# PixelClear/OclPathTracer

Measured on AMD Instinct MI355X. Metric: Msamples/sec (pixels x spp / s), cornellbox.bin 1024x1024, higher is better.
Workload: dtype f32; 1 GPU; BASELINE configs[2]: cornellbox.bin 1024x1024, 256 spp, depth 16, full path; render_lanes=2, checkpointed_launches=True, staging_ring_bytes=402653184, workspace_bytes=510711120

## Files before the change

### include/pt_shim.h

```cpp
#ifndef PT_SHIM_H
#define PT_SHIM_H

#include <stddef.h>
#include <stdint.h>

#ifdef __cplusplus
extern "C" {
#endif

#define PT_SHIM_ABI_VERSION 2

enum pt_status {
    PT_OK = 0,
    PT_ERR_INVALID = 1,
    PT_ERR_NO_DEVICE = 2,
    PT_ERR_OOM = 3,
    PT_ERR_HIP = 4,
    PT_ERR_NOT_FOUND = 5,
    PT_ERR_ARGS = 6,
    PT_ERR_RANGE = 7,
    PT_ERR_TRAVERSAL = 8
};

typedef struct pt_device_s* pt_device_t;
// ... 368 lines not shown
                 const pt_reproject_params* params, const pt_camera* prev_cam, const pt_camera* cur_cam ,
                 pt_event_t ev);

enum { PT_PROF_TRACE = 0, PT_PROF_FOLD = 1, PT_PROF_KINDS = 2 };
int pt_profile_enable(pt_device_t dev, int on);
int pt_profile_query(pt_device_t dev, int kind, double* total_ms, uint64_t* launches);
int pt_profile_query_union(pt_device_t dev, int kind, double* union_ms);
int pt_profile_reset(pt_device_t dev);

#define PT_BVH_SNAPSHOT_BIG_MAX 64
typedef struct pt_bvh_info {
    uint32_t records;
    int32_t num_big;
    int32_t num_triangles;
    float grid_min[3], grid_step[3];
    int32_t reserved[7];
} pt_bvh_info;
int pt_bvh_snapshot(pt_device_t dev, pt_bvh_info* info, void* records, size_t record_capacity, int32_t* big_indices);

int pt_primary_mask_snapshot(pt_device_t dev, uint32_t* num_pixels, void* masks, size_t capacity);

int pt_secondary_mask_snapshot(pt_device_t dev, uint32_t info[4], void* masks, size_t capacity);

int pt_assemble_stripes(pt_device_t dev, pt_buffer_t gathered, pt_buffer_t image, int width,
                        int height, int stripe_rows, int n_ranks, int slab_rows, pt_event_t ev);

int pt_assemble_stripes_on(pt_device_t dev, pt_buffer_t gathered, pt_buffer_t image, int width, int height,
                           int stripe_rows, int n_ranks, int slab_rows, void* hip_stream);

int pt_tonemap_ppm(pt_device_t dev, pt_buffer_t framebuffer, pt_buffer_t rgb_i32, size_t num_pixels,
                   pt_event_t ev);

#ifdef __cplusplus
}
#endif
#endif
```

### oclpathtracer_amd/csrc/pt_kernels.h

```cpp
#pragma once

#include <hip/hip_runtime.h>
#include <stddef.h>
#include <stdint.h>

struct PtRawTriangle { float p1[4], p2[4], p3[4]; int32_t id; char pad[12]; };
struct PtRawMaterial { float albedo[4], emissive[4]; float roughness; int32_t type; char pad[24]; };
static_assert(sizeof(PtRawTriangle) == 64 && sizeof(PtRawMaterial) == 64, "record layout");

struct PtPrepTriangle {
    float p1[3];
    float e1[3];
    float e2[3];
    float pad0[3];
    float n[3];
    int32_t id;
};
static_assert(sizeof(PtPrepTriangle) == 64, "prep layout");

struct PtBvhNode {
    float lmin[3]; uint32_t link_l;
    float lmax[3]; uint32_t link_r;
    float rmin[3]; uint32_t pad0;
    float rmax[3]; uint32_t pad1;
// ... 51 lines not shown
    uint32_t rad1_off;
    int32_t max_bounces, ntri, nmat;
    int32_t stripe_rows, n_ranks, rank;
    uint32_t npix_local;
    uint32_t batches_per_frame, total_batches;
    uint32_t batch;
    float quad_delta1;
    float ray_radius;
    const float* p1tab;
    float p1_lo, p1_hi;
    const PtBvh8Node* bvh;
    int32_t bvh_records;
    PtBvhGrid grid;
    const PtPrepTriangle* bigtab;
    const int32_t* bigidx;
    int32_t nbig;
    const uint2* pmask;
    unsigned int* bvh_flags;
    int32_t bvh_stack_limit;
    uint32_t* carry;
    uint32_t carry_in_waves;
    uint32_t carry_out;
    PtCamera cam;
    const uint2* smask;
};
#define PT_QUEUE_SHARDS 8
#define PT_QUEUE_SHARD_WORDS 1056
#define PT_QUEUE_STOP_WORD (PT_QUEUE_SHARDS * PT_QUEUE_SHARD_WORDS)
#define PT_QUEUE_WORDS ((PT_QUEUE_SHARDS + 1) * PT_QUEUE_SHARD_WORDS)
#define PT_POOL 56
#define PT_CARRY_RECORDS 64
#define PT_CARRY_STRIDE_DW (16 + PT_CARRY_RECORDS * 15)
#define PT_CARRY_HIT_RECORDS PT_POOL
#define PT_CARRY_HIT_STRIDE_DW (16 + PT_CARRY_HIT_RECORDS * 18)
static_assert(PT_CARRY_HIT_STRIDE_DW >= PT_CARRY_STRIDE_DW, "a checkpoint region holds either kernel's records");
static_assert(PT_CARRY_HIT_STRIDE_DW % 4 == 0 && PT_CARRY_STRIDE_DW % 4 == 0, "a region's float4 arrays begin 16 dwords in: every region 16-byte aligned");
#define PT_PACKED_BOUNCE_MAX 256

struct PtFoldParams {
    const float* rad;
    float4* fb;
    uint32_t npix_local;
    int32_t frame_begin, frame_count;
    unsigned int* reset_counter;
    unsigned int* reset_counter2;
};

#define PT_PREP_WORDS 12
__host__ __device__ static inline unsigned ptk_order_key(float f)
{
    unsigned u;
    __builtin_memcpy(&u, &f, sizeof u);
    return (u & 0x80000000u) ? ~u : (u | 0x80000000u);
}
__host__ __device__ static inline float ptk_order_float(unsigned k)
{
    const unsigned u = (k & 0x80000000u) ? (k & 0x7fffffffu) : ~k;
    float f;
    __builtin_memcpy(&f, &u, sizeof f);
    return f;
}
hipError_t ptk_prep_triangles(const PtRawTriangle* raw, PtPrepTriangle* out, int ntri, unsigned int* det_bound_bits,
                              hipStream_t s);
hipError_t ptk_prep_quad_margins(PtPrepTriangle* out, int ntri, float diameter, float delta1, float* p1tab, const float anchor[3], hipStream_t s);
#define PT_P1_STRIDE 24
static inline size_t ptk_p1tab_floats(int ntri) { return (size_t)((ntri / 2 + 1) / 2) * PT_P1_STRIDE; }
hipError_t ptk_primary_masks(const PtTraceParams& p, hipStream_t s);
hipError_t ptk_secondary_masks(const PtPrepTriangle* tris, int ntri, uint2* table, hipStream_t s);
struct PtSearchMode {
    bool bvh;
    bool det_bounded;
    int quads;
};
hipError_t ptk_trace(const PtTraceParams& p, int num_blocks, PtSearchMode m, bool tally, bool wide, hipStream_t s);
#define PT_BVH_NEAR_EYE 4.0f
hipError_t ptk_bvh_big_raw(const PtRawTriangle* raw, const int* bigidx, int nbig, PtRawTriangle* out, hipStream_t s);
static inline size_t ptk_bvh_record_count(int ntri) { return 2 * (size_t)(ntri > 0 ? ntri : 0); }
size_t ptk_bvh_temp_bytes(int ntri);
#define PT_BVH_BIG_MAX 64
#define PT_BVH_RAY_EPS 1.2e-4f
hipError_t ptk_bvh_build(const PtRawTriangle* raw, const PtPrepTriangle* prep, int ntri, PtBvh8Node* recs,
                         PtPrepTriangle* bigtab, int* bigidx, int* nbig_dev, PtBvhGrid* grid_dev, unsigned* used_dev, void* temp, size_t temp_bytes,
                         hipStream_t s);
#define PT_DET_BOUND_MAX 2.0e19f
#define PT_BVH_AUTO_MIN 512
hipError_t ptk_fold(const PtFoldParams& p, hipStream_t s);
hipError_t ptk_assemble_stripes(const float4* gathered, float4* image, int width, int height, int stripe_rows,
                                int n_ranks, int slab_rows, hipStream_t s);
hipError_t ptk_tonemap_ppm(const float4* fb, int32_t* rgb, size_t npix, hipStream_t s);
hipError_t ptk_fill_i32(int32_t* dst, int32_t value, int n, hipStream_t s);
hipError_t ptk_math(const float* in, float* out, int n, hipStream_t s);
// ... 167 lines not shown
```

### oclpathtracer_amd/csrc/pt_kernels.hip

```cpp
#include "pt_kernels.h"

#include "pt_device_math.h"
#include "pt_secmask.h"

#include <type_traits>
#include <utility>

typedef const __attribute__((address_space(4))) float* pt_const_f32p;

PTK_DEV unsigned pt_lane_id() { return __builtin_amdgcn_mbcnt_hi(~0u, __builtin_amdgcn_mbcnt_lo(~0u, 0u)); }
PTK_DEV unsigned pt_mbcnt(unsigned long long m) { return __builtin_amdgcn_mbcnt_hi((unsigned)(m >> 32), __builtin_amdgcn_mbcnt_lo((unsigned)m, 0u)); }

typedef const __attribute__((address_space(4))) PtTraceParams* pt_kargs_p;
PTK_DEV pt_kargs_p pt_kargs()
{
    pt_kargs_p k = (pt_kargs_p)__builtin_amdgcn_kernarg_segment_ptr();
    asm volatile("" : "+s"(k));
    return k;
}
PTK_DEV f3 pt_anchor()
{
    const pt_kargs_p K = pt_kargs();
    return mk3(K->cam.eye[0], K->cam.eye[1], K->cam.eye[2]);
}
// ... 220 lines not shown
    for (int j = 0; j < P.ntri; ++j) {
        const PtPrepTriangle* t = P.tris + j;
        const f3 e1 = mk3(t->e1[0], t->e1[1], t->e1[2]), e2 = mk3(t->e2[0], t->e2[1], t->e2[2]);
        const f3 tv = mk3(o.x - t->p1[0], o.y - t->p1[1], o.z - t->p1[2]);
        const f3 Kd = cross3(e2, e1), Ku = cross3(e2, tv), qv = cross3(tv, e1);
        const float tn = dot3(e2, qv);
        const float detc = dot3(dc, Kd), unc = dot3(dc, Ku), vnc = dot3(dc, qv);
        const float a1 = pt_norm1(e1), a2 = pt_norm1(e2), at = pt_norm1(tv);
        const float rho_d = (eps * pt_norm1(Kd) + uS * (a1 * a2)) * 1.001f + A;
        const float rho_u = (eps * pt_norm1(Ku) + uS * (at * a2)) * 1.001f + A;
        const float rho_v = (eps * pt_norm1(qv) + uS * (at * a1)) * 1.001f + A;
        const bool keep = !(detc + rho_d < 0.999e-8f)
                        & !(unc + rho_u < 0.0f)
                        & !(vnc + rho_v < 0.0f)
                        & !((unc - rho_u) + (vnc - rho_v) > (detc + rho_d) * 1.000002f)
                        & !(tn <= 0.0f);
        const int c = j >> 5;
        const int nc = P.ntri - 32 * c < 32 ? P.ntri - 32 * c : 32;
        m[c] |= (keep ? 1u : 0u) << (nc - 1 - (j & 31));
    }
    P.out[lp] = make_uint2(m[0], m[1]);
}

__global__ __launch_bounds__(256) void pt_secondary_mask_kernel(const PtPrepTriangle* tris, int ntri, uint2* table)
{
    const unsigned i = blockIdx.x * blockDim.x + threadIdx.x;
    if (i < (unsigned)ntri) reinterpret_cast<PtSmTri*>(table)[i] = pt_sm_tri_record(tris[i].p1, tris[i].e1, tris[i].e2);
    if (i >= (unsigned)ntri * PT_SM_TRI_ENTRIES) return;
    const unsigned k = i / PT_SM_TRI_ENTRIES, within = i - k * PT_SM_TRI_ENTRIES;
    const unsigned dir = within / (PT_SM_T * PT_SM_T), tile = within - dir * (PT_SM_T * PT_SM_T);
    const unsigned e = k * PT_SM_TRI_ENTRIES + tile * PT_SM_DIRS + dir;
    const PtSmMask m = pt_sm_entry(reinterpret_cast<const float*>(tris), ntri, e);
    table[PT_SM_HEAD_ENTRIES + e] = make_uint2(m.x, m.y);
}

struct PtTriRec { float p1x, p1y, p1z, e1x, e1y, e1z, e2x, e2y, e2z; };

PTK_DEV PtTriRec pt_load_tri(pt_const_f32p T, int i)
{
    pt_const_f32p t = T + 16 * i;
    PtTriRec r;
    r.p1x = t[0]; r.p1y = t[1]; r.p1z = t[2];
    r.e1x = t[3]; r.e1y = t[4]; r.e1z = t[5];
    r.e2x = t[6]; r.e2y = t[7]; r.e2z = t[8];
    return r;
}

#ifndef PT_VALIDATE_FILTER
#define PT_VALIDATE_FILTER 0
#endif
typedef unsigned long long pt_lanes;
#define PT_LANES(cond) __builtin_amdgcn_ballot_w64(cond)
#define PT_ON(mask) __builtin_amdgcn_inverse_ballot_w64(mask)
PTK_DEV unsigned pt_push_flag(unsigned m, pt_lanes c)
{
    unsigned long long carry_out;
// ... 1068 lines not shown
            if (primary && P.pmask != nullptr) {
                pm = P.pmask[pix0 + lane];
                masked = true;
            } else if (LDS_TABLE == 1 && PT_TRACE_SECONDARY_MASKS && !fresh) {
                const pt_kargs_p KS = pt_kargs();
                const uint2* const sm = KS->smask;
                const int nt = KS->ntri;
                if (sm != nullptr) {
#if PT_STAMPS
                    unsigned long long ta = 0, tb = 0;
                    PT_STAMP(ta);
#endif
                    const PtSmMask ones = pt_sm_all_ones(nt);
                    pm = make_uint2(ones.x, ones.y);
                    if (PT_ON(alive)) {
                        const char* const base = reinterpret_cast<const char*>(sm);
                        const unsigned k = (unsigned)h.hidx < (unsigned)(nt - 1) ? (unsigned)h.hidx : (unsigned)(nt - 1);
                        const float4 ra = *reinterpret_cast<const float4*>(base + (size_t)(k * 48u));
                        const float4 rb = *reinterpret_cast<const float4*>(base + (size_t)(k * 48u + 16u));
                        const float4 rn = *reinterpret_cast<const float4*>(base + (size_t)(k * 48u + 32u));
                        const float A[4] = { ra.x, ra.y, ra.z, ra.w }, B[4] = { rb.x, rb.y, rb.z, rb.w }, N[4] = { rn.x, rn.y, rn.z, rn.w };
                        unsigned entry;
                        const bool covered = pt_sm_classify(A, B, N, s.o.x, s.o.y, s.o.z, s.d.x, s.d.y, s.d.z, k, &entry);
                        const uint2 v = *reinterpret_cast<const uint2*>(base + (size_t)(entry * 8u + (unsigned)(PT_SM_HEAD_ENTRIES * 8)));
                        if (covered) pm = v;
#if PT_VALIDATE_FILTER
                        if (P.stats) {
                            const pt_lanes unc = PT_LANES(!covered);
                            if (lane == (unsigned)__builtin_ctzll(alive)) {
                                atomicAdd(&P.stats[10], (unsigned long long)__popcll(alive));
                                atomicAdd(&P.stats[11], (unsigned long long)__popcll(unc & alive));
                            }
                        }
#endif
                    }
                    masked = true;
#if PT_STAMPS
                    PT_STAMP(tb);
                    c_p1 += tb - ta;
#endif
                }
            }
        }
        if (alive == 0ull) {
        } else if (masked)
            p2steps = pt_intersect_masked<DET_BOUNDED, LDS_TABLE>(T, P.tris, ntri, s.o, s.d, PT_ON(alive), tmax, hu, hv, hidx, pm, tl, lane,
                                                                  PT_VALIDATE_FILTER && P.stats ? P.stats + 2 : nullptr);
// ... 2671 lines not shown
    const int pairs = ntri / 2;
    hipLaunchKernelGGL(pt_prep_quad_margins_kernel, dim3((pairs + 255) / 256), dim3(256), 0, s, out, ntri, diameter, delta1);
    if (p1tab) {
        const int qpairs = (pairs + 1) / 2;
        hipLaunchKernelGGL(pt_prep_p1tab_kernel, dim3((qpairs + 255) / 256), dim3(256), 0, s, out, ntri, diameter, p1tab, anchor[0], anchor[1], anchor[2]);
    }
    return hipGetLastError();
}

hipError_t ptk_primary_masks(const PtTraceParams& p, hipStream_t s)
{
    if (!p.pmask || p.npix_local == 0) return hipSuccess;
    PtMaskParams m;
    m.tris = p.tris;
    m.out = const_cast<uint2*>(p.pmask);
    m.width = p.width; m.height = p.height; m.ntri = p.ntri;
    m.stripe_rows = p.stripe_rows; m.n_ranks = p.n_ranks; m.rank = p.rank;
    m.npix_local = p.npix_local;
    m.cam = p.cam;
    hipLaunchKernelGGL(pt_primary_mask_kernel, dim3((p.npix_local + 255u) / 256u), dim3(256), 0, s, m);
    return hipGetLastError();
}

hipError_t ptk_secondary_masks(const PtPrepTriangle* tris, int ntri, uint2* table, hipStream_t s)
{
    if (!table || ntri <= 0 || ntri > PT_SM_TRI_MAX) return hipErrorInvalidValue;
    const unsigned n = (unsigned)ntri * PT_SM_TRI_ENTRIES;
    hipLaunchKernelGGL(pt_secondary_mask_kernel, dim3((n + 255u) / 256u), dim3(256), 0, s, tris, ntri, table);
    return hipGetLastError();
}

hipError_t ptk_trace(const PtTraceParams& p, int num_blocks, PtSearchMode m, bool tally, bool wide, hipStream_t s)
{
    const bool q3 = m.quads == 3;
    void (*kernel)(const PtTraceParams);
    if (m.bvh && wide)
        kernel = tally ? (m.det_bounded ? (q3 ? pt_trace_bvh_kernel<true, true, 3, true> : pt_trace_bvh_kernel<true, true, 0, true>) : pt_trace_bvh_kernel<false, true, 0, true>)
                       : (m.det_bounded ? (q3 ? pt_trace_bvh_kernel<true, false, 3, true> : pt_trace_bvh_kernel<true, false, 0, true>) : pt_trace_bvh_kernel<false, false, 0, true>);
    else if (m.bvh)
        kernel = tally ? (m.det_bounded ? (q3 ? pt_trace_bvh_kernel<true, true, 3> : pt_trace_bvh_kernel<true, true, 0>) : pt_trace_bvh_kernel<false, true, 0>)
                       : (m.det_bounded ? (q3 ? pt_trace_bvh_kernel<true, false, 3> : pt_trace_bvh_kernel<true, false, 0>) : pt_trace_bvh_kernel<false, false, 0>);
    else if (p.ntri <= PT_LDS_TRI_MAX)
        kernel = m.det_bounded ? (q3 ? pt_trace_kernel<true, 1, 3> : pt_trace_kernel<true, 1, 0>) : pt_trace_kernel<false, 1, 0>;
    else
        kernel = m.det_bounded ? pt_trace_tiled_kernel<true> : pt_trace_tiled_kernel<false>;
    const size_t lds = m.bvh ? ptk_trace_bvh_lds_bytes() : ptk_trace_lds_bytes(p.ntri);
    hipLaunchKernelGGL(kernel, dim3(num_blocks), dim3(PT_TRACE_THREADS), lds, s, p);
    return hipGetLastError();
}

hipError_t ptk_fold(const PtFoldParams& p, hipStream_t s)
// ... 278 lines not shown
```

### oclpathtracer_amd/csrc/pt_secmask.h

```cpp
#pragma once

#include <math.h>
#include <stdint.h>

#if defined(__HIPCC__)
#define PT_SM_HD __host__ __device__ static inline
#else
#define PT_SM_HD static inline
#endif

#ifndef PT_SM_T
#define PT_SM_T 12
#endif
#ifndef PT_SM_C
#define PT_SM_C 11
#endif
#ifndef PT_SM_DEPTH
#define PT_SM_DEPTH 3
#endif
#ifndef PT_SM_BUDGET
#define PT_SM_BUDGET 96
#endif
#ifndef PT_SM_SEP_DET
#define PT_SM_SEP_DET 1e-4
#endif
#define PT_SM_GUARD (1.0 / 64.0)
#define PT_SM_DIRS (6 * PT_SM_C * PT_SM_C)
#define PT_SM_TRI_ENTRIES (PT_SM_T * PT_SM_T * PT_SM_DIRS)
#define PT_SM_TRI_MAX 64
struct PtSmTri { float A[4], B[4], N[4]; };
#define PT_SM_HEAD_ENTRIES (PT_SM_TRI_MAX * sizeof(PtSmTri) / 8)
#define PT_SM_TABLE_BYTES(ntri) ((PT_SM_HEAD_ENTRIES + (size_t)(ntri) * PT_SM_TRI_ENTRIES) * 8)
static_assert(PT_SM_T >= 1 && PT_SM_C >= 1 && PT_SM_C <= 16, "pt_sm_classify's rounding bound is derived for C <= 16");
static_assert(PT_SM_TABLE_BYTES(PT_SM_TRI_MAX) < 0x100000000ull, "an entry's byte offset in the largest table must fit 32 bits");

struct PtSmMask { unsigned x, y; };

PT_SM_HD float pt_sm_form(const float* F, float ox, float oy, float oz)
{
    return __builtin_fmaf(F[2], oz, __builtin_fmaf(F[1], oy, __builtin_fmaf(F[0], ox, F[3])));
}

PT_SM_HD bool pt_sm_classify(const float* A, const float* B, const float* N, float ox, float oy, float oz, float dx, float dy, float dz,
                             unsigned k, unsigned* entry)
{
    const float tu = pt_sm_form(A, ox, oy, oz), tv = pt_sm_form(B, ox, oy, oz), th = pt_sm_form(N, ox, oy, oz);
    const float dd = __builtin_fmaf(dz, dz, __builtin_fmaf(dy, dy, dx * dx));
    const bool covered = (tu >= 0.0f) & (tu < (float)PT_SM_T) & (tv >= 0.0f) & (tv < (float)PT_SM_T) & (__builtin_fabsf(th) <= 1.0f) &
                         (dd >= 0.999f) & (dd <= 1.001f);
    const float ax = __builtin_fabsf(dx), ay = __builtin_fabsf(dy), az = __builtin_fabsf(dz);
    const bool mx = (ax >= ay) & (ax >= az), my = ay >= az;
    const unsigned m = mx ? 0u : my ? 1u : 2u;
    const float dm = mx ? dx : my ? dy : dz;
    const float da = mx ? dy : my ? dz : dx;
    const float db = mx ? dz : my ? dx : dy;
#if defined(__HIP_DEVICE_COMPILE__)
    const float r = __builtin_amdgcn_rcpf(__builtin_fabsf(dm));
// ... 55 lines not shown
    pt_sm_form_make(pt_sm_v(as.x / nn, as.y / nn, as.z / nn), G, st, reach, g.p1, g.rec.A, &Eu);
    pt_sm_form_make(pt_sm_v(bs.x / nn, bs.y / nn, bs.z / nn), G, st, reach, g.p1, g.rec.B, &Ev);
    pt_sm_form_make(g.nh, 0.0, 1.0 / g.H, reach, g.p1, g.rec.N, &Eh);
    g.du = 8.0 * PT_SM_U * Eu; g.dv = 8.0 * PT_SM_U * Ev; g.dh = 8.0 * PT_SM_U * Eh;
    bool ok = nn > 0.0 && g.du <= 0.25 && g.dv <= 0.25 && g.dh <= 0.25;
    ok = ok && 0.0101 * sqrt(pt_sm_dot(as, as)) / nn <= G && 0.0101 * sqrt(pt_sm_dot(bs, bs)) / nn <= G;
    for (int i = 0; i < 4; ++i)
        ok = ok && fabs((double)g.rec.A[i]) < 1e30 && fabs((double)g.rec.B[i]) < 1e30 && fabs((double)g.rec.N[i]) < 1e30;
    g.valid = ok;
    if (!ok)
        for (int i = 0; i < 4; ++i) g.rec.A[i] = g.rec.B[i] = g.rec.N[i] = __builtin_nanf("");
    return g;
}

PT_SM_HD PtSmTri pt_sm_tri_record(const float* p1, const float* e1, const float* e2) { return pt_sm_geom(p1, e1, e2).rec; }

PT_SM_HD PtSmMask pt_sm_all_ones(int ntri)
{
    PtSmMask m;
    const int n0 = ntri < 32 ? ntri : 32, n1 = ntri - 32 < 0 ? 0 : ntri - 32 > 32 ? 32 : ntri - 32;
    m.x = n0 == 32 ? ~0u : (1u << n0) - 1u;
    m.y = n1 == 32 ? ~0u : (1u << n1) - 1u;
    return m;
}

PT_SM_HD void pt_sm_ratio_range(int i, double* lo, double* hi)
{
    const double dc = 1e-4;
    *lo = fmax(-1.0, ((double)i - dc) * (2.0 / PT_SM_C) - 1.0);
    *hi = fmin(1.0, ((double)i + 1.0 + dc) * (2.0 / PT_SM_C) - 1.0);
}
PT_SM_HD double pt_sm_absmin(double lo, double hi) { return lo > 0.0 ? lo : hi < 0.0 ? -hi : 0.0; }
PT_SM_HD double pt_sm_absmax(double lo, double hi) { return fmax(fabs(lo), fabs(hi)); }
PT_SM_HD void pt_sm_set(PtSmV3* v, unsigned axis, double x) { if (axis == 0u) v->x = x; else if (axis == 1u) v->y = x; else v->z = x; }

PT_SM_HD bool pt_sm_keep(const PtSmGeom& g, PtSmV3 oc, double ru, double rv, double Hr, PtSmV3 dc, PtSmV3 rd, const float* tj)
{
    const double INF = 1.001, ABS = 2e-24, RHO = 32.0 * PT_SM_U;
    const PtSmV3 q1 = pt_sm_vf(tj), f1 = pt_sm_vf(tj + 3), f2 = pt_sm_vf(tj + 6);
    const PtSmV3 tc = pt_sm_sub(oc, q1);
    const double f1n = pt_sm_n1(f1), f2n = pt_sm_n1(f2);
    const double tv1 = pt_sm_n1(tc) + ru * pt_sm_n1(g.e1) + rv * pt_sm_n1(g.e2) + 3.0 * Hr;
    const PtSmV3 Kd = pt_sm_cross(f2, f1);
    const double det_hi = pt_sm_dot(dc, Kd) + ((pt_sm_absdot(rd, Kd) + RHO * f1n * f2n) * INF + ABS);
    if (det_hi < 0.999e-8) return false;
    const PtSmV3 Gt = pt_sm_cross(f1, f2);
// ... 155 lines not shown
```

### oclpathtracer_amd/csrc/pt_shim.hip

```cpp
#include "../../include/pt_shim.h"

#include <hip/hip_runtime.h>

#include <algorithm>
#include <cmath>
#include <cstdarg>
#include <cstdio>
#include <cstdlib>
#include <cstring>
#include <initializer_list>
#include <new>
#include <string>
#include <utility>
#include <vector>

#include "pt_denoise.h"
#include "pt_reproject.h"
#include "pt_kernels.h"
#include "pt_secmask.h"

static thread_local char g_err[512] = "";

static int fail(int code, const char* fmt, ...)
{
// ... 96 lines not shown
    bool bvh_valid;
    uint64_t bvh_builds;
    int bvh_blocks_per_cu;
    int query_bvh_blocks_per_cu;
    int lit_bvh_blocks_per_cu[PT_LIT_KINDS];
    unsigned int* trav_host;
    unsigned int* trav_dev;
    PtWs<float> ring;
    size_t ring_slot_bytes;
    hipStream_t lane[2];
    hipEvent_t ev_fork;
    hipEvent_t ev_fold[2];
    hipEvent_t ev_slot[2];
    hipEvent_t ev_ext;
    bool fold_recorded[2], slot_recorded[2];
    int last_fold_lane;
    bool lanes_busy;
    bool main_dirty;
    uint64_t chunk_seq, render_seq;
    PtWs<uint32_t> carry[2];
    PtWs<uint2> pmask;
    struct { uint64_t scene_gen; int32_t g[7]; PtCamera cam; bool valid; } pmask_key;
    PtWs<uint2> smask;
    struct { uint64_t scene_gen; int32_t ntri; bool valid, declined; } smask_key;
    PtWs<unsigned int> counters;
    bool counters_dirty;
    bool prof_on;
    std::vector<std::pair<hipEvent_t, hipEvent_t>> prof_pairs[PT_PROF_KINDS];
    size_t prof_used[PT_PROF_KINDS];
};

#define PT_RING_SLOTS 2
#define PT_DEFAULT_SLOT_BYTES ((size_t)192 << 20)
#define PT_QUEUE_COUNTERS 64
#define PT_QUEUE_STRIDE PT_QUEUE_WORDS

static int prof_begin(pt_device_s* d, int kind, hipStream_t st, hipEvent_t* stop_out)
{
    *stop_out = nullptr;
    if (!d->prof_on) return PT_OK;
    auto& v = d->prof_pairs[kind];
    if (d->prof_used[kind] == v.size()) {
        hipEvent_t a, b;
        HIP_TRY(hipEventCreate(&a));
        HIP_TRY(hipEventCreate(&b));
        v.push_back({ a, b });
    }
// ... 348 lines not shown
        return rc;
    case PT_OPT_CHUNK_FRAMES:
        if (value < 0) return fail(PT_ERR_INVALID, "chunk frames must be >= 0");
        d->opt_chunk = value;
        return PT_OK;
    case PT_OPT_PROFILE_RETURN_TIME:
        d->opt_profile = value ? 1 : 0;
        return PT_OK;
    case PT_OPT_QUAD_FILTER:
        if (value < 0 || value > 4) return fail(PT_ERR_INVALID, "quad filter must be 0 (auto), 1..3 (independent triangles) or 4 (packed shared u)");
        d->opt_quads = value;
        return PT_OK;
    case PT_OPT_ACCEL:
        if (value < 0 || value > 2) return fail(PT_ERR_INVALID, "accel must be 0 (auto), 1 (brute force) or 2 (BVH)");
        d->opt_accel = value;
        return PT_OK;
    case PT_OPT_BVH_TALLY:
        d->opt_tally = value ? 1 : 0;
        return PT_OK;
    case PT_OPT_PRIMARY_MASKS:
        d->opt_pmask = value ? 1 : 0;
        return PT_OK;
    case PT_OPT_SECONDARY_MASKS:
        d->opt_smask = value ? 1 : 0;
        return PT_OK;
    case PT_OPT_DENOISE_TILE:
        if (value < 0 || value > 2) return fail(PT_ERR_INVALID, "the denoiser's gather must be 0 (auto), 1 (global loads) or 2 (LDS tile at steps 1 and 2)");
        d->opt_denoise = value;
        return PT_OK;
    case PT_OPT_REPROJECT_FORM:
        if (value < 0 || value > 2) return fail(PT_ERR_INVALID, "the reprojection's form must be 0 (auto), 1 (one kernel over the records) or 2 (a prepare pass first)");
        d->opt_reproject = value;
        return PT_OK;
    case PT_OPT_BVH_STACK_LIMIT:
        if (value < 1 || value > 64) return fail(PT_ERR_INVALID, "the LBVH stack limit must be 1..64");
        d->opt_bvh_stack = value;
        return PT_OK;
    case PT_OPT_RENDER_LANES:
        if (value < 1 || value > 2) return fail(PT_ERR_INVALID, "render lanes must be 1 or 2");
        rc = enter_stream(d);
        d->opt_lanes = value;
        return rc;
    case PT_OPT_CHECKPOINT:
        d->opt_carry = value ? 1 : 0;
        return PT_OK;
    case PT_OPT_RESERVED_3:
        if (value != 0 && value != 1) return fail(PT_ERR_INVALID, "option 3 took 0 or 1");
// ... 640 lines not shown
}

static int refresh_pmask(pt_device_s* d, const pt_render_params& rp, const PtCamera& cam, uint32_t npix, bool& make)
{
    int rc;
    const int32_t g[7] = { rp.width, rp.height, rp.stripe_rows, rp.n_ranks, rp.rank, (int32_t)npix, rp.num_triangles };
    make = !d->pmask_key.valid || d->pmask_key.scene_gen != d->scene_gen || memcmp(d->pmask_key.g, g, sizeof g) != 0 ||
           memcmp(&d->pmask_key.cam, &cam, sizeof cam) != 0;
    if (!make) return PT_OK;
    if ((rc = stream_enqueue(d))) return rc;
    d->pmask_key.valid = false;
    if (d->pmask.bytes < (size_t)npix * sizeof(uint2)) {
        HIP_TRY(hipStreamSynchronize(d->stream));
        ws_free(d, d->pmask);
        hipError_t e = ws_malloc(d, d->pmask, (size_t)npix * sizeof(uint2));
        if (e != hipSuccess) return fail(PT_ERR_OOM, "primary-mask allocation (%zu bytes) failed: %s", (size_t)npix * sizeof(uint2), hipGetErrorString(e));
    }
    d->pmask_key.scene_gen = d->scene_gen;
    memcpy(d->pmask_key.g, g, sizeof g);
    d->pmask_key.cam = cam;
    return PT_OK;
}

static int refresh_smask(pt_device_s* d, int ntri)
{
    int rc;
    if ((d->smask_key.valid || d->smask_key.declined) && d->smask_key.scene_gen == d->scene_gen && d->smask_key.ntri == ntri) return PT_OK;
    if ((rc = stream_enqueue(d))) return rc;
    d->smask_key.valid = d->smask_key.declined = false;
    {
        PtPrepTriangle host[PT_SM_TRI_MAX];
        HIP_TRY(hipMemcpyAsync(host, d->prep.p, (size_t)ntri * sizeof(PtPrepTriangle), hipMemcpyDeviceToHost, d->stream));
        HIP_TRY(hipStreamSynchronize(d->stream));
        bool all = true;
        for (int k = 0; k < ntri && all; ++k) all = pt_sm_geom(host[k].p1, host[k].e1, host[k].e2).valid;
        d->smask_key.scene_gen = d->scene_gen;
        d->smask_key.ntri = ntri;
        d->smask_key.declined = !all;
        if (!all) return PT_OK;
    }
    if (d->smask.bytes < PT_SM_TABLE_BYTES(ntri)) {
        HIP_TRY(hipStreamSynchronize(d->stream));
        ws_free(d, d->smask);
        hipError_t e = ws_malloc(d, d->smask, PT_SM_TABLE_BYTES(ntri));
        if (e != hipSuccess) return fail(PT_ERR_OOM, "secondary-mask allocation (%zu bytes) failed: %s", (size_t)PT_SM_TABLE_BYTES(ntri), hipGetErrorString(e));
    }
    HIP_TRY(ptk_secondary_masks(d->prep, ntri, d->smask, d->stream));
    d->smask_key.scene_gen = d->scene_gen;
    d->smask_key.ntri = ntri;
    d->smask_key.valid = true;
    return PT_OK;
}

static bool pmask_footprint_holds(int width, int height)
{
    return (double)width * width + (double)height * height <= 7626.0 * 7626.0;
}

static int choose_batch(const pt_device_s* d, bool use_bvh, uint32_t npix, int chunk, uint32_t& batch, uint32_t& bpf, int& blocks)
{
    const int wg_waves = PT_TRACE_THREADS / 64;
    blocks = d->prop.multiProcessorCount * (use_bvh ? d->bvh_blocks_per_cu : d->blocks_per_cu);
    const uint64_t resident_waves = (uint64_t)blocks * wg_waves;
    const uint64_t chunk_samples = (uint64_t)npix * (uint64_t)chunk;
    batch = PT_TRACE_BATCH;
    while (batch > 128u && chunk_samples / batch < 64u * resident_waves) batch >>= 1;
    bpf = (npix + batch - 1) / batch;
    if ((uint64_t)bpf * (uint64_t)chunk + PT_QUEUE_SHARDS > 0xffffffffull) return fail(PT_ERR_INVALID, "chunk too large");
    const uint64_t blocks_needed = ((uint64_t)bpf * (uint64_t)chunk + wg_waves - 1) / wg_waves;
    if ((uint64_t)blocks > blocks_needed) blocks = (int)blocks_needed;
    return PT_OK;
}
// ... 42 lines not shown
    return PT_OK;
}

static int render_part(pt_device_s* d, pt_buffer_s* tris, pt_buffer_s* mats, pt_buffer_s* fb, const pt_render_params& rp, const PtCamera& cam,
                       uint32_t npix, pt_buffer_s* stats, pt_event_s* ev_start, pt_event_s* ev_stop)
{
    int rc;
    PtSearch search;
    if ((rc = prepare_search(d, tris, rp.num_triangles, cam.eye, search))) return rc;
    const bool use_bvh = search.mode.bvh;
    if (!use_bvh && rp.num_triangles <= PT_LDS_TRI_MAX && rp.max_bounces > PT_PACKED_BOUNCE_MAX)
        return fail(PT_ERR_INVALID, "max_bounces above %d on a scene of at most %d triangles without the LBVH (a parked path packs its bounce count in 8 bits)",
                    PT_PACKED_BOUNCE_MAX, PT_LDS_TRI_MAX);
    int nchunks, chunk;
    if ((rc = plan_chunks(d, rp.frame_count, npix, nchunks, chunk))) return rc;
    const bool want_pmask = d->opt_pmask && search.mode.quads == 3 && !use_bvh && rp.num_triangles <= 64 && search.mode.det_bounded;
    const bool use_pmask = want_pmask && pmask_footprint_holds(rp.width, rp.height);
    if (want_pmask && !use_pmask) d->pmask_key.valid = false;
    bool make_pmask = false;
    if (use_pmask && (rc = refresh_pmask(d, rp, cam, npix, make_pmask))) return rc;
    const bool can_smask = search.mode.quads == 3 && !use_bvh && rp.num_triangles <= PT_SM_TRI_MAX && search.mode.det_bounded;
    const bool use_smask = can_smask && d->opt_smask;
    if (!can_smask) d->smask_key.valid = d->smask_key.declined = false;
    if (use_smask && (rc = refresh_smask(d, rp.num_triangles))) return rc;
    if (d->counters_dirty) {
        if ((rc = stream_enqueue(d))) return rc;
        HIP_TRY(hipMemsetAsync(d->counters, 0, WS_COUNTERS, d->stream));
        d->counters_dirty = false;
    }
    uint32_t batch, bpf;
    int blocks;
    if ((rc = choose_batch(d, use_bvh, npix, chunk, batch, bpf, blocks))) return rc;
    PtTraceParams tp = trace_params(d, mats, stats, rp, cam, npix, search, use_pmask, chunk, batch, bpf);
    tp.smask = use_smask && d->smask_key.valid ? d->smask.p : nullptr;
    if (make_pmask) {
        HIP_TRY(ptk_primary_masks(tp, d->stream));
        d->pmask_key.valid = true;
    }
    const bool carry = d->opt_carry != 0 && nchunks > 1;
    int ln = d->opt_lanes == 2 ? (int)(d->render_seq++ & 1u) : 0;
    hipStream_t st = d->lane[ln];
    if (carry && (rc = ensure_carry(d, blocks))) return rc;
    const int wg_waves = PT_TRACE_THREADS / 64;

    if (d->main_dirty || d->external) {
        HIP_TRY(hipEventRecord(d->ev_fork, d->stream));
        HIP_TRY(hipStreamWaitEvent(d->lane[0], d->ev_fork, 0));
        HIP_TRY(hipStreamWaitEvent(d->lane[1], d->ev_fork, 0));
        d->main_dirty = false;
    }
    d->lanes_busy = true;
    d->counters_dirty = true;
    if (ev_start) HIP_TRY(hipEventRecord(ev_start->start, st));
    tp.ring_phase = (uint32_t)((d->chunk_seq & 1u) ? chunk : 0);
    tp.carry = carry ? d->carry[ln].p : nullptr;
    unsigned int* const drain_counter = d->counters + (size_t)(PT_QUEUE_COUNTERS - 1 - ln) * PT_QUEUE_STRIDE;
    unsigned int* prev_counter = nullptr;
// ... 1168 lines not shown
    if (!d->pmask_key.valid || d->pmask_key.scene_gen != d->scene_gen || !d->pmask.p)
        return fail(PT_ERR_INVALID, "no primary-ray masks stand for the prepared scene");
    const size_t npix = (size_t)(uint32_t)d->pmask_key.g[5];
    *num_pixels = (uint32_t)npix;
    if (masks) {
        if (capacity < npix) return fail(PT_ERR_RANGE, "pt_primary_mask_snapshot: %zu pixels do not fit %zu", npix, capacity);
        if (npix) HIP_TRY(hipMemcpy(masks, d->pmask.p, npix * sizeof(uint2), hipMemcpyDeviceToHost));
    }
    return PT_OK;
}

extern "C" int pt_secondary_mask_snapshot(pt_device_t d, uint32_t info[4], void* masks, size_t capacity)
{
    int rc = use_device(d);
    if (rc) return rc;
    if (!info) return fail(PT_ERR_INVALID, "pt_secondary_mask_snapshot: info is null");
    if ((rc = flush_pending(d)) || (rc = stream_wait(d))) return rc;
    if (!d->smask_key.valid || d->smask_key.scene_gen != d->scene_gen || d->smask_key.ntri != d->prep_ntri || !d->smask.p)
        return fail(PT_ERR_INVALID, "no secondary-ray masks stand for the prepared scene");
    const size_t n = (size_t)d->smask_key.ntri * PT_SM_TRI_ENTRIES;
    info[0] = (uint32_t)n; info[1] = (uint32_t)d->smask_key.ntri; info[2] = PT_SM_T; info[3] = PT_SM_C;
    if (masks) {
        if (capacity < n) return fail(PT_ERR_RANGE, "pt_secondary_mask_snapshot: %zu entries do not fit %zu", n, capacity);
        HIP_TRY(hipMemcpy(masks, d->smask.p + PT_SM_HEAD_ENTRIES, n * sizeof(uint2), hipMemcpyDeviceToHost));
    }
    return PT_OK;
}

extern "C" int pt_profile_query_union(pt_device_t d, int kind, double* union_ms)
{
    int rc = use_device(d);
    if (rc) return rc;
    if (kind < 0 || kind >= PT_PROF_KINDS || !union_ms) return fail(PT_ERR_INVALID, "bad profile query");
    if ((rc = enter_stream(d)) || (rc = stream_wait(d))) return rc;
    const size_t n = d->prof_used[kind];
    std::vector<std::pair<double, double>> iv(n);
    for (size_t i = 0; i < n; ++i) {
        float a = 0.f, b = 0.f;
        if (i) HIP_TRY(hipEventElapsedTime(&a, d->prof_pairs[kind][0].first, d->prof_pairs[kind][i].first));
        HIP_TRY(hipEventElapsedTime(&b, d->prof_pairs[kind][0].first, d->prof_pairs[kind][i].second));
        iv[i] = { (double)a, (double)b };
    }
    std::sort(iv.begin(), iv.end());
    double total = 0.0, end = -1.0e300;
    for (auto& x : iv) {
        if (x.second <= end) continue;
        total += x.second - std::max(x.first, end);
        end = x.second;
// ... 188 lines not shown
```

### oclpathtracer_amd/shim.py

```python
from __future__ import annotations

import ctypes
import os

_HERE = os.path.dirname(os.path.abspath(__file__))
LIB_PATH = os.environ.get("PT_SHIM_LIB") or os.path.join(_HERE, "libptshim.so")

PT_OK = 0
PT_ERR_INVALID, PT_ERR_NO_DEVICE, PT_ERR_OOM, PT_ERR_HIP, PT_ERR_NOT_FOUND, PT_ERR_ARGS, PT_ERR_RANGE, PT_ERR_TRAVERSAL = range(1, 9)
PT_INFO_NAME, PT_INFO_BOARD, PT_INFO_VENDOR, PT_INFO_VERSION = range(4)
PT_OPT_BATCH_FRAMES, PT_OPT_CHUNK_FRAMES, PT_OPT_PROFILE_RETURN_TIME = 0, 1, 2
PT_OPT_QUAD_FILTER, PT_OPT_ACCEL, PT_OPT_BVH_TALLY, PT_OPT_PRIMARY_MASKS, PT_OPT_BVH_STACK_LIMIT, PT_OPT_RENDER_LANES, PT_OPT_CHECKPOINT, PT_OPT_BVH_BUILD_COUNT = 4, 5, 6, 7, 8, 9, 10, 11
PT_OPT_SECONDARY_MASKS = 12
PT_OPT_DENOISE_TILE = 13
PT_OPT_REPROJECT_FORM = 14
PT_SHIM_ABI_VERSION = 2
PT_MAX_ARG_SIZE = 64
PT_MAX_ARG_COUNT = 64
PT_STAT_SAMPLES, PT_STAT_RAYS, PT_STAT_WORDS = 0, 1, 16
PT_STAT_BVH_NODES, PT_STAT_BVH_TRIS, PT_STAT_BVH_STEPS, PT_STAT_BVH_TRI_STEPS, PT_STAT_BVH_MAX_STACK, PT_STAT_CARRIED, PT_STAT_BVH_GRAZING = 2, 3, 4, 5, 6, 7, 8
PT_PROF_TRACE, PT_PROF_FOLD = 0, 1
PT_STREAM_LEGACY = 1
PT_QUERY_CLOSEST, PT_QUERY_OCCLUDED = 0, 1

# ... 273 lines not shown
                                             _c.POINTER(Roulette), _c.POINTER(Camera), _H]),
    "pt_render_direct_ris": (_c.c_int, [_H, _H, _H, _H, _H, _H, _H, _H, _c.POINTER(DirectParams), _c.POINTER(Ris), _c.POINTER(Camera), _H]),
    "pt_render_indirect_ris": (_c.c_int, [_H, _H, _H, _H, _c.c_int, _H, _H, _H, _H, _H, _c.POINTER(IndirectParams), _c.POINTER(Roulette),
                                          _c.POINTER(Ris), _c.POINTER(Camera), _H]),
    "pt_render_indirect_pixels_ris": (_c.c_int, [_H, _H, _H, _H, _c.c_int, _H, _H, _H, _H, _H, _H, _c.c_uint32, _c.POINTER(IndirectParams),
                                                 _c.POINTER(Roulette), _c.POINTER(Ris), _c.POINTER(Camera), _H]),
    "pt_sample_moments_pixels": (_c.c_int, [_H, _H, _H, _H, _c.c_uint32, _c.c_int32, _H]),
    "pt_env_table_bytes": (_c.c_size_t, [_c.c_int]),
    "pt_env_table": (_c.c_int, [_H, _H, _c.c_int, _H, _H]),
    "pt_render_direct_env": (_c.c_int, [_H, _H, _H, _H, _H, _H, _H, _H, _H, _H, _c.POINTER(DirectParams), _c.POINTER(Environment),
                                        _c.POINTER(Camera), _H]),
    "pt_render_indirect_env": (_c.c_int, [_H, _H, _H, _H, _H, _H, _H, _H, _H, _H, _H, _c.POINTER(IndirectParams), _c.POINTER(Roulette),
                                          _c.POINTER(Environment), _c.POINTER(Camera), _H]),
    "pt_radiance_rays": (_c.c_int, [_H, _H, _H, _H, _c.c_int, _H, _H, _H, _H, _H, _H, _c.POINTER(RadianceParams), _c.POINTER(Roulette), _H]),
    "pt_denoise_scratch_bytes": (_c.c_size_t, [_c.c_int32, _c.c_int32]),
    "pt_denoise": (_c.c_int, [_H, _H, _H, _H, _H, _H, _H, _H, _c.POINTER(DenoiseParams), _H]),
    "pt_reproject_scratch_bytes": (_c.c_size_t, [_c.c_int32, _c.c_int32]),
    "pt_reproject": (_c.c_int, [_H, _H, _H, _H, _H, _H, _H, _H, _H, _c.POINTER(ReprojectParams), _c.POINTER(Camera), _c.POINTER(Camera), _H]),
    "pt_profile_enable": (_c.c_int, [_H, _c.c_int]),
    "pt_profile_query": (_c.c_int, [_H, _c.c_int, _c.POINTER(_c.c_double), _c.POINTER(_c.c_uint64)]),
    "pt_bvh_snapshot": (_c.c_int, [_H, _c.POINTER(BvhInfo), _c.c_void_p, _c.c_size_t, _c.c_void_p]),
    "pt_primary_mask_snapshot": (_c.c_int, [_H, _c.POINTER(_c.c_uint32), _c.c_void_p, _c.c_size_t]),
    "pt_secondary_mask_snapshot": (_c.c_int, [_H, _c.POINTER(_c.c_uint32), _c.c_void_p, _c.c_size_t]),
    "pt_profile_query_union": (_c.c_int, [_H, _c.c_int, _c.POINTER(_c.c_double)]),
    "pt_profile_reset": (_c.c_int, [_H]),
    "pt_assemble_stripes": (_c.c_int, [_H, _H, _H, _c.c_int, _c.c_int, _c.c_int, _c.c_int, _c.c_int, _H]),
    "pt_assemble_stripes_on": (_c.c_int, [_H, _H, _H, _c.c_int, _c.c_int, _c.c_int, _c.c_int, _c.c_int, _c.c_void_p]),
    "pt_tonemap_ppm": (_c.c_int, [_H, _H, _H, _c.c_size_t, _H]),
}


class ShimError(RuntimeError):
    def __init__(self, code: int, message: str):
        super().__init__("pt_shim error %d: %s" % (code, message))
        self.code = code


_lib = None


def load():
    global _lib
    if _lib is None:
        if not os.path.exists(LIB_PATH):
            raise ShimError(PT_ERR_NO_DEVICE, "libptshim.so is not built (run __graft_entry__.build()); "
                                              "there is no CPU fallback for the hot path")
# ... 16 lines not shown
```

Baseline: 10730 Msamples/s.

## Compress secondary-ray mask table with a hashed mask dictionary and finer tiling

Replaces the per-entry 8-byte secondary mask table with 2- or 4-byte indices into a deduplicated dictionary of distinct masks, built by a GPU hash-intern kernel. It also raises the tile and direction resolution (T 12→17, C 11→15), so masks are finer and cull more triangles. Lookups gain an extra dependent load, and the build now needs a host sync and may retry with the wide form or decline when the dictionary overflows.

```diff
diff --git a/include/pt_shim.h b/include/pt_shim.h
--- a/include/pt_shim.h
+++ b/include/pt_shim.h
@@ -414,6 +414,8 @@
 
 int pt_secondary_mask_snapshot(pt_device_t dev, uint32_t info[4], void* masks, size_t capacity);
 
+int pt_secondary_mask_format(pt_device_t dev, uint64_t format[5]);
+
 int pt_assemble_stripes(pt_device_t dev, pt_buffer_t gathered, pt_buffer_t image, int width,
                         int height, int stripe_rows, int n_ranks, int slab_rows, pt_event_t ev);
 
diff --git a/oclpathtracer_amd/csrc/pt_kernels.h b/oclpathtracer_amd/csrc/pt_kernels.h
--- a/oclpathtracer_amd/csrc/pt_kernels.h
+++ b/oclpathtracer_amd/csrc/pt_kernels.h
@@ -97,8 +97,10 @@
     uint32_t carry_in_waves;
     uint32_t carry_out;
     PtCamera cam;
+    uint32_t smask_dict;
     const uint2* smask;
 };
+static_assert(sizeof(PtTraceParams) == 328 && offsetof(PtTraceParams, smask) == 320, "smask_dict took padding: every kernel's argument offsets are what they were");
 #define PT_QUEUE_SHARDS 8
 #define PT_QUEUE_SHARD_WORDS 1056
 #define PT_QUEUE_STOP_WORD (PT_QUEUE_SHARDS * PT_QUEUE_SHARD_WORDS)
@@ -141,7 +143,7 @@
 #define PT_P1_STRIDE 24
 static inline size_t ptk_p1tab_floats(int ntri) { return (size_t)((ntri / 2 + 1) / 2) * PT_P1_STRIDE; }
 hipError_t ptk_primary_masks(const PtTraceParams& p, hipStream_t s);
-hipError_t ptk_secondary_masks(const PtPrepTriangle* tris, int ntri, uint2* table, hipStream_t s);
+hipError_t ptk_secondary_masks(const PtPrepTriangle* tris, int ntri, uint2* table, bool wide, hipStream_t s);
 struct PtSearchMode {
     bool bvh;
     bool det_bounded;
diff --git a/oclpathtracer_amd/csrc/pt_kernels.hip b/oclpathtracer_amd/csrc/pt_kernels.hip
--- a/oclpathtracer_amd/csrc/pt_kernels.hip
+++ b/oclpathtracer_amd/csrc/pt_kernels.hip
@@ -266,7 +266,15 @@
     P.out[lp] = make_uint2(m[0], m[1]);
 }
 
-__global__ __launch_bounds__(256) void pt_secondary_mask_kernel(const PtPrepTriangle* tris, int ntri, uint2* table)
+__global__ __launch_bounds__(256) void pt_secondary_mask_init_kernel(unsigned char* table, int ntri, unsigned dict_off, unsigned slots)
+{
+    unsigned long long* const dict = reinterpret_cast<unsigned long long*>(table + dict_off);
+    const unsigned i = blockIdx.x * blockDim.x + threadIdx.x;
+    if (i < slots) pt_sm_dict_init_slot(dict, i, ntri);
+    if (i == 0u) { unsigned* const status = reinterpret_cast<unsigned*>(dict + slots); status[0] = 0u; status[1] = 1u; }
+}
+
+__global__ __launch_bounds__(256) void pt_secondary_mask_kernel(const PtPrepTriangle* tris, int ntri, unsigned char* table, unsigned dict_off, unsigned slots)
 {
     const unsigned i = blockIdx.x * blockDim.x + threadIdx.x;
     if (i < (unsigned)ntri) reinterpret_cast<PtSmTri*>(table)[i] = pt_sm_tri_record(tris[i].p1, tris[i].e1, tris[i].e2);
@@ -275,7 +283,14 @@
     const unsigned dir = within / (PT_SM_T * PT_SM_T), tile = within - dir * (PT_SM_T * PT_SM_T);
     const unsigned e = k * PT_SM_TRI_ENTRIES + tile * PT_SM_DIRS + dir;
     const PtSmMask m = pt_sm_entry(reinterpret_cast<const float*>(tris), ntri, e);
-    table[PT_SM_HEAD_ENTRIES + e] = make_uint2(m.x, m.y);
+    unsigned long long* const dict = reinterpret_cast<unsigned long long*>(table + dict_off);
+    unsigned* const status = reinterpret_cast<unsigned*>(dict + slots);
+    bool fresh;
+    unsigned slot = pt_sm_intern(dict, slots, ntri, m, &fresh);
+    if (fresh) atomicAdd(status + 1, 1u);
+    if (slot == slots) { status[0] = 1u; slot = 0u; }
+    if (slots == PT_SM_WIDE_SLOTS) reinterpret_cast<unsigned*>(table + PT_SM_HEAD_BYTES)[e] = slot;
+    else reinterpret_cast<unsigned short*>(table + PT_SM_HEAD_BYTES)[e] = (unsigned short)slot;
 }
 
 struct PtTriRec { float p1x, p1y, p1z, e1x, e1y, e1z, e2x, e2y, e2z; };
@@ -1390,7 +1405,11 @@
                         const float A[4] = { ra.x, ra.y, ra.z, ra.w }, B[4] = { rb.x, rb.y, rb.z, rb.w }, N[4] = { rn.x, rn.y, rn.z, rn.w };
                         unsigned entry;
                         const bool covered = pt_sm_classify(A, B, N, s.o.x, s.o.y, s.o.z, s.d.x, s.d.y, s.d.z, k, &entry);
-                        const uint2 v = *reinterpret_cast<const uint2*>(base + (size_t)(entry * 8u + (unsigned)(PT_SM_HEAD_ENTRIES * 8)));
+                        const unsigned form = KS->smask_dict;
+                        unsigned ix;
+                        if (__builtin_expect((form & 1u) != 0u, 0)) ix = *reinterpret_cast<const unsigned*>(base + (size_t)(entry * 4u + (unsigned)PT_SM_HEAD_BYTES));
+                        else ix = *reinterpret_cast<const unsigned short*>(base + (size_t)(entry * 2u + (unsigned)PT_SM_HEAD_BYTES));
+                        const uint2 v = *reinterpret_cast<const uint2*>(base + (size_t)(ix * 8u + (form & ~1u)));
                         if (covered) pm = v;
 #if PT_VALIDATE_FILTER
                         if (P.stats) {
@@ -4108,11 +4127,13 @@
     return hipGetLastError();
 }
 
-hipError_t ptk_secondary_masks(const PtPrepTriangle* tris, int ntri, uint2* table, hipStream_t s)
+hipError_t ptk_secondary_masks(const PtPrepTriangle* tris, int ntri, uint2* table, bool wide, hipStream_t s)
 {
     if (!table || ntri <= 0 || ntri > PT_SM_TRI_MAX) return hipErrorInvalidValue;
-    const unsigned n = (unsigned)ntri * PT_SM_TRI_ENTRIES;
-    hipLaunchKernelGGL(pt_secondary_mask_kernel, dim3((n + 255u) / 256u), dim3(256), 0, s, tris, ntri, table);
+    const unsigned n = (unsigned)ntri * PT_SM_TRI_ENTRIES, slots = PT_SM_DICT_SLOTS(wide), dict_off = (unsigned)PT_SM_DICT_OFFSET(ntri, wide);
+    unsigned char* const t = reinterpret_cast<unsigned char*>(table);
+    hipLaunchKernelGGL(pt_secondary_mask_init_kernel, dim3((slots + 255u) / 256u), dim3(256), 0, s, t, ntri, dict_off, slots);
+    hipLaunchKernelGGL(pt_secondary_mask_kernel, dim3((n + 255u) / 256u), dim3(256), 0, s, tris, ntri, t, dict_off, slots);
     return hipGetLastError();
 }
 
diff --git a/oclpathtracer_amd/csrc/pt_secmask.h b/oclpathtracer_amd/csrc/pt_secmask.h
--- a/oclpathtracer_amd/csrc/pt_secmask.h
+++ b/oclpathtracer_amd/csrc/pt_secmask.h
@@ -10,10 +10,10 @@
 #endif
 
 #ifndef PT_SM_T
-#define PT_SM_T 12
+#define PT_SM_T 17
 #endif
 #ifndef PT_SM_C
-#define PT_SM_C 11
+#define PT_SM_C 15
 #endif
 #ifndef PT_SM_DEPTH
 #define PT_SM_DEPTH 3
@@ -29,10 +29,19 @@
 #define PT_SM_TRI_ENTRIES (PT_SM_T * PT_SM_T * PT_SM_DIRS)
 #define PT_SM_TRI_MAX 64
 struct PtSmTri { float A[4], B[4], N[4]; };
-#define PT_SM_HEAD_ENTRIES (PT_SM_TRI_MAX * sizeof(PtSmTri) / 8)
-#define PT_SM_TABLE_BYTES(ntri) ((PT_SM_HEAD_ENTRIES + (size_t)(ntri) * PT_SM_TRI_ENTRIES) * 8)
+#define PT_SM_HEAD_BYTES (PT_SM_TRI_MAX * sizeof(PtSmTri))
+#define PT_SM_NARROW_SLOTS 65536u
+#define PT_SM_WIDE_SLOTS (1u << 21)
+#define PT_SM_STATUS_BYTES 8
+#define PT_SM_INDEX_BYTES(wide) ((wide) ? 4u : 2u)
+#define PT_SM_DICT_SLOTS(wide) ((wide) ? PT_SM_WIDE_SLOTS : PT_SM_NARROW_SLOTS)
+#define PT_SM_DICT_OFFSET(ntri, wide) ((PT_SM_HEAD_BYTES + (size_t)(ntri) * PT_SM_TRI_ENTRIES * PT_SM_INDEX_BYTES(wide) + 7) / 8 * 8)
+#define PT_SM_STATUS_OFFSET(ntri, wide) (PT_SM_DICT_OFFSET(ntri, wide) + (size_t)PT_SM_DICT_SLOTS(wide) * 8)
+#define PT_SM_TABLE_BYTES(ntri, wide) (PT_SM_STATUS_OFFSET(ntri, wide) + PT_SM_STATUS_BYTES)
 static_assert(PT_SM_T >= 1 && PT_SM_C >= 1 && PT_SM_C <= 16, "pt_sm_classify's rounding bound is derived for C <= 16");
-static_assert(PT_SM_TABLE_BYTES(PT_SM_TRI_MAX) < 0x100000000ull, "an entry's byte offset in the largest table must fit 32 bits");
+static_assert(PT_SM_TABLE_BYTES(PT_SM_TRI_MAX, 1) < 0x100000000ull && PT_SM_TABLE_BYTES(PT_SM_TRI_MAX, 0) < 0x100000000ull,
+              "a byte offset in the largest table (64 triangles, wide form) must fit 32 bits");
+static_assert(PT_SM_HEAD_BYTES % 8 == 0 && PT_SM_NARROW_SLOTS == 1u << 16, "the dictionary is 8-byte aligned; a 2-byte index names any narrow slot");
 
 struct PtSmMask { unsigned x, y; };
 
@@ -134,6 +143,46 @@
     m.x = n0 == 32 ? ~0u : (1u << n0) - 1u;
     m.y = n1 == 32 ? ~0u : (1u << n1) - 1u;
     return m;
+}
+
+#define PT_SM_EMPTY 0xffffffffffffffffull
+PT_SM_HD unsigned long long pt_sm_word(PtSmMask m) { return (unsigned long long)m.x | ((unsigned long long)m.y << 32); }
+PT_SM_HD PtSmMask pt_sm_unword(unsigned long long w) { PtSmMask m = { (unsigned)w, (unsigned)(w >> 32) }; return m; }
+PT_SM_HD unsigned pt_sm_hash(unsigned long long w)
+{
+    w ^= w >> 33; w *= 0xff51afd7ed558ccdull; w ^= w >> 33; w *= 0xc4ceb9fe1a85ec53ull; w ^= w >> 33;
+    return (unsigned)w;
+}
+PT_SM_HD void pt_sm_dict_init_slot(unsigned long long* dict, unsigned slot, int ntri) { dict[slot] = slot == 0u ? pt_sm_word(pt_sm_all_ones(ntri)) : PT_SM_EMPTY; }
+PT_SM_HD unsigned pt_sm_intern(unsigned long long* dict, unsigned capacity, int ntri, PtSmMask m, bool* fresh)
+{
+    const unsigned long long w = pt_sm_word(m);
+    *fresh = false;
+    if (w == pt_sm_word(pt_sm_all_ones(ntri))) return 0u;
+    const unsigned span = capacity - 1u;
+    unsigned at = pt_sm_hash(w) % span;
+    for (unsigned i = 0; i < span; ++i) {
+        unsigned long long* const slot = dict + 1u + at;
+#if defined(__HIP_DEVICE_COMPILE__)
+        unsigned long long seen = __hip_atomic_load(slot, __ATOMIC_RELAXED, __HIP_MEMORY_SCOPE_AGENT);
+        if (seen == PT_SM_EMPTY) {
+            seen = atomicCAS(slot, PT_SM_EMPTY, w);
+            if (seen == PT_SM_EMPTY) { *fresh = true; return 1u + at; }
+        }
+#else
+        unsigned long long seen = *slot;
+        if (seen == PT_SM_EMPTY) { *slot = w; *fresh = true; return 1u + at; }
+#endif
+        if (seen == w) return 1u + at;
+        at = at + 1u == span ? 0u : at + 1u;
+    }
+    return capacity;
+}
+PT_SM_HD PtSmMask pt_sm_decode(const unsigned char* table, int ntri, bool wide, unsigned entry)
+{
+    const unsigned char* const ix = table + PT_SM_HEAD_BYTES;
+    const unsigned i = wide ? reinterpret_cast<const unsigned*>(ix)[entry] : (unsigned)reinterpret_cast<const unsigned short*>(ix)[entry];
+    return pt_sm_unword(reinterpret_cast<const unsigned long long*>(table + PT_SM_DICT_OFFSET(ntri, wide))[i]);
 }
 
 PT_SM_HD void pt_sm_ratio_range(int i, double* lo, double* hi)
diff --git a/oclpathtracer_amd/csrc/pt_shim.hip b/oclpathtracer_amd/csrc/pt_shim.hip
--- a/oclpathtracer_amd/csrc/pt_shim.hip
+++ b/oclpathtracer_amd/csrc/pt_shim.hip
@@ -142,7 +142,7 @@
     PtWs<uint2> pmask;
     struct { uint64_t scene_gen; int32_t g[7]; PtCamera cam; bool valid; } pmask_key;
     PtWs<uint2> smask;
-    struct { uint64_t scene_gen; int32_t ntri; bool valid, declined; } smask_key;
+    struct { uint64_t scene_gen; int32_t ntri; bool valid, declined, forced, wide; uint32_t retries, used; } smask_key;
     PtWs<unsigned int> counters;
     bool counters_dirty;
     bool prof_on;
@@ -537,7 +537,7 @@
         d->opt_pmask = value ? 1 : 0;
         return PT_OK;
     case PT_OPT_SECONDARY_MASKS:
-        d->opt_smask = value ? 1 : 0;
+        d->opt_smask = value == 2 ? 2 : value ? 1 : 0;
         return PT_OK;
     case PT_OPT_DENOISE_TILE:
         if (value < 0 || value > 2) return fail(PT_ERR_INVALID, "the denoiser's gather must be 0 (auto), 1 (global loads) or 2 (LDS tile at steps 1 and 2)");
@@ -1224,12 +1224,15 @@
     return PT_OK;
 }
 
-static int refresh_smask(pt_device_s* d, int ntri)
+static int refresh_smask(pt_device_s* d, int ntri, bool forced)
 {
     int rc;
-    if ((d->smask_key.valid || d->smask_key.declined) && d->smask_key.scene_gen == d->scene_gen && d->smask_key.ntri == ntri) return PT_OK;
+    if ((d->smask_key.valid || d->smask_key.declined) && d->smask_key.scene_gen == d->scene_gen && d->smask_key.ntri == ntri && d->smask_key.forced == forced)
+        return PT_OK;
     if ((rc = stream_enqueue(d))) return rc;
     d->smask_key.valid = d->smask_key.declined = false;
+    d->smask_key.forced = forced;
+    d->smask_key.retries = d->smask_key.used = 0;
     {
         PtPrepTriangle host[PT_SM_TRI_MAX];
         HIP_TRY(hipMemcpyAsync(host, d->prep.p, (size_t)ntri * sizeof(PtPrepTriangle), hipMemcpyDeviceToHost, d->stream));
@@ -1241,15 +1244,28 @@
         d->smask_key.declined = !all;
         if (!all) return PT_OK;
     }
-    if (d->smask.bytes < PT_SM_TABLE_BYTES(ntri)) {
+    for (bool wide = forced;; wide = true) {
+        const size_t need = PT_SM_TABLE_BYTES(ntri, wide);
+        if (d->smask.bytes != need) {
+            HIP_TRY(hipStreamSynchronize(d->stream));
+            ws_free(d, d->smask);
+            hipError_t e = ws_malloc(d, d->smask, need);
+            if (e != hipSuccess) return fail(PT_ERR_OOM, "secondary-mask allocation (%zu bytes) failed: %s", need, hipGetErrorString(e));
+        }
+        HIP_TRY(ptk_secondary_masks(d->prep, ntri, d->smask, wide, d->stream));
+        uint32_t status[2] = { 0u, 0u };
+        HIP_TRY(hipMemcpyAsync(status, reinterpret_cast<const char*>(d->smask.p) + PT_SM_STATUS_OFFSET(ntri, wide), sizeof status, hipMemcpyDeviceToHost, d->stream));
         HIP_TRY(hipStreamSynchronize(d->stream));
-        ws_free(d, d->smask);
-        hipError_t e = ws_malloc(d, d->smask, PT_SM_TABLE_BYTES(ntri));
-        if (e != hipSuccess) return fail(PT_ERR_OOM, "secondary-mask allocation (%zu bytes) failed: %s", (size_t)PT_SM_TABLE_BYTES(ntri), hipGetErrorString(e));
-    }
-    HIP_TRY(ptk_secondary_masks(d->prep, ntri, d->smask, d->stream));
-    d->smask_key.scene_gen = d->scene_gen;
-    d->smask_key.ntri = ntri;
+        d->smask_key.wide = wide;
+        d->smask_key.used = status[1];
+        if (!status[0]) break;
+        d->smask_key.retries++;
+        if (wide) {
+            d->smask_key.declined = true;
+            (void)fail(PT_OK, "secondary masks declined: the scene's %d triangles have more distinct masks than the wide dictionary's %u slots", ntri, PT_SM_WIDE_SLOTS);
+            return PT_OK;
+        }
+    }
     d->smask_key.valid = true;
     return PT_OK;
 }
@@ -1338,7 +1354,7 @@
     const bool can_smask = search.mode.quads == 3 && !use_bvh && rp.num_triangles <= PT_SM_TRI_MAX && search.mode.det_bounded;
     const bool use_smask = can_smask && d->opt_smask;
     if (!can_smask) d->smask_key.valid = d->smask_key.declined = false;
-    if (use_smask && (rc = refresh_smask(d, rp.num_triangles))) return rc;
+    if (use_smask && (rc = refresh_smask(d, rp.num_triangles, d->opt_smask == 2))) return rc;
     if (d->counters_dirty) {
         if ((rc = stream_enqueue(d))) return rc;
         HIP_TRY(hipMemsetAsync(d->counters, 0, WS_COUNTERS, d->stream));
@@ -1349,6 +1365,7 @@
     if ((rc = choose_batch(d, use_bvh, npix, chunk, batch, bpf, blocks))) return rc;
     PtTraceParams tp = trace_params(d, mats, stats, rp, cam, npix, search, use_pmask, chunk, batch, bpf);
     tp.smask = use_smask && d->smask_key.valid ? d->smask.p : nullptr;
+    tp.smask_dict = tp.smask ? (uint32_t)PT_SM_DICT_OFFSET(rp.num_triangles, d->smask_key.wide) | (d->smask_key.wide ? 1u : 0u) : 0u;
     if (make_pmask) {
         HIP_TRY(ptk_primary_masks(tp, d->stream));
         d->pmask_key.valid = true;
@@ -2563,8 +2580,29 @@
     info[0] = (uint32_t)n; info[1] = (uint32_t)d->smask_key.ntri; info[2] = PT_SM_T; info[3] = PT_SM_C;
     if (masks) {
         if (capacity < n) return fail(PT_ERR_RANGE, "pt_secondary_mask_snapshot: %zu entries do not fit %zu", n, capacity);
-        HIP_TRY(hipMemcpy(masks, d->smask.p + PT_SM_HEAD_ENTRIES, n * sizeof(uint2), hipMemcpyDeviceToHost));
-    }
+        const bool wide = d->smask_key.wide;
+        std::vector<unsigned char> table(PT_SM_TABLE_BYTES(d->smask_key.ntri, wide));
+        HIP_TRY(hipMemcpy(table.data(), d->smask.p, table.size(), hipMemcpyDeviceToHost));
+        PtSmMask* const out = static_cast<PtSmMask*>(masks);
+        for (size_t e = 0; e < n; ++e) out[e] = pt_sm_decode(table.data(), d->smask_key.ntri, wide, (unsigned)e);
+    }
+    return PT_OK;
+}
+
+extern "C" int pt_secondary_mask_format(pt_device_t d, uint64_t format[5])
+{
+    int rc = use_device(d);
+    if (rc) return rc;
+    if (!format) return fail(PT_ERR_INVALID, "pt_secondary_mask_format: format is null");
+    if ((rc = flush_pending(d)) || (rc = stream_wait(d))) return rc;
+    if (!d->smask_key.valid || d->smask_key.scene_gen != d->scene_gen || d->smask_key.ntri != d->prep_ntri || !d->smask.p)
+        return fail(PT_ERR_INVALID, "no secondary-ray masks stand for the prepared scene");
+    const bool wide = d->smask_key.wide;
+    format[0] = PT_SM_INDEX_BYTES(wide);
+    format[1] = PT_SM_DICT_SLOTS(wide);
+    format[2] = d->smask_key.used;
+    format[3] = PT_SM_TABLE_BYTES(d->smask_key.ntri, wide);
+    format[4] = d->smask_key.retries;
     return PT_OK;
 }
 
diff --git a/oclpathtracer_amd/shim.py b/oclpathtracer_amd/shim.py
--- a/oclpathtracer_amd/shim.py
+++ b/oclpathtracer_amd/shim.py
@@ -319,6 +319,7 @@
     "pt_bvh_snapshot": (_c.c_int, [_H, _c.POINTER(BvhInfo), _c.c_void_p, _c.c_size_t, _c.c_void_p]),
     "pt_primary_mask_snapshot": (_c.c_int, [_H, _c.POINTER(_c.c_uint32), _c.c_void_p, _c.c_size_t]),
     "pt_secondary_mask_snapshot": (_c.c_int, [_H, _c.POINTER(_c.c_uint32), _c.c_void_p, _c.c_size_t]),
+    "pt_secondary_mask_format": (_c.c_int, [_H, _c.POINTER(_c.c_uint64)]),
     "pt_profile_query_union": (_c.c_int, [_H, _c.c_int, _c.POINTER(_c.c_double)]),
     "pt_profile_reset": (_c.c_int, [_H]),
     "pt_assemble_stripes": (_c.c_int, [_H, _H, _H, _c.c_int, _c.c_int, _c.c_int, _c.c_int, _c.c_int, _H]),
```

New measurement: 10590 Msamples/s. -1.3%, worse.
